# pangenome/povu

Measured on AMD Instinct MI355X. Metric: edges/sec decomposed (flubble+PVST), higher is better.
Workload: dtype u32

## Files before the change

include/povu_hip.h:

```cpp
#ifndef POVU_HIP_H
#define POVU_HIP_H

#include <stddef.h>
#include <stdint.h>

#ifdef __cplusplus
extern "C" {
#endif

#define POVU_HIP_NIL 0xFFFFFFFFu
#define POVU_SIDE_L 0
#define POVU_SIDE_R 1
#define POVU_TIP_NONE 0
#define POVU_TIP_L 1
#define POVU_TIP_R 2

typedef struct povu_hip_ctx povu_hip_ctx;
typedef struct povu_hip_forest povu_hip_forest;

int povu_hip_device_count(void);

povu_hip_ctx *povu_hip_create(int device, char *err, size_t errlen);
void povu_hip_destroy(povu_hip_ctx *ctx);
int povu_hip_release_workspace(povu_hip_ctx *ctx);
// ... 191 lines not shown
uint32_t povu_hip_last_seq_redo(const povu_hip_ctx *ctx);
int povu_hip_last_black_only_classes(const povu_hip_ctx *ctx);
int povu_hip_last_laminar_check_ran(const povu_hip_ctx *ctx);
int povu_hip_last_crossings(povu_hip_ctx *ctx, uint32_t out[2]);
uint64_t povu_hip_last_links_processed(const povu_hip_ctx *ctx);

int povu_hip_debug_components(povu_hip_ctx *ctx, uint32_t *comp_of, uint32_t *local_idx);
int povu_hip_debug_tree(povu_hip_ctx *ctx, uint32_t comp, uint32_t *n_tree, uint32_t *gid, uint8_t *typ,
			uint32_t *par, uint32_t *cls);
int povu_hip_debug_edge_ids(povu_hip_ctx *ctx, uint32_t comp, uint32_t *n_tree, uint32_t *tree_edge_id);
int povu_hip_debug_stack(povu_hip_ctx *ctx, uint32_t comp, uint32_t *n, uint32_t *tree_vtx, uint32_t *cls,
			 uint32_t *next_seen);

int povu_hip_debug_scan(povu_hip_ctx *ctx, int op, const uint32_t *in, uint32_t *out, size_t n, const uint32_t *in2,
			uint32_t *out2, size_t n2);
double povu_hip_debug_scan_time(povu_hip_ctx *ctx, size_t n, int reps, int op);

uint64_t povu_hip_workspace_estimate(uint32_t n_vtx, uint32_t n_links, uint32_t n_components);
int povu_hip_workspace_breakdown(uint32_t n_vtx, uint32_t n_links, uint32_t n_components, uint64_t out[7]);
int povu_hip_prewarm(povu_hip_ctx *ctx, uint32_t n_vtx, uint32_t n_links, char *err, size_t errlen);
uint64_t povu_hip_leaf_workspace_estimate(uint32_t n_vtx, uint32_t n_components);

const char *povu_hip_version(void);

#ifdef __cplusplus
}
#endif
#endif
```

povu_amd/csrc/hip/povu_hip.hip:

```cpp
#include "context.hpp"

#include <algorithm>
#include <atomic>
#include <cstdlib>
#include <memory>
#include <mutex>
#include <numeric>
#include <type_traits>

#include <fcntl.h>
#include <sys/mman.h>
#include <unistd.h>

using namespace povu_hip;

PinnedPool::~PinnedPool()
{
	for (auto &b : free_blocks)
		if (b.seg < 0)
			(void)hipHostFree(b.p);
	for (auto &sg : segments) {
		(void)hipHostUnregister(sg.p);
		(void)munmap(sg.p, sg.cap);
		(void)shm_unlink(segment_name(shared_tag, sg.seg).c_str());
// ... 1574 lines not shown
			scan_exclusive_u32_pair(di, dout, n, di2, dout2, n2, tmp, tb, s);
		else if (op == 0)
			scan_exclusive_u32(di, dout, n, tmp, tb, s);
		else
			scan_exclusive_max_u32(di, dout, n, tmp, tb, s);
		HIP_CHECK(copy_async(out, dout, n * 4, hipMemcpyDeviceToHost, s));
		if (in2 && op == 0)
			HIP_CHECK(copy_async(out2, dout2, n2 * 4, hipMemcpyDeviceToHost, s));
		HIP_CHECK(hipStreamSynchronize(s));
		return 0;
	} catch (const std::exception &) {
		return 2;
	}
}

extern "C" double povu_hip_debug_scan_time(povu_hip_ctx *ctx, size_t n, int reps, int op)
{
	if (!ctx || !n || reps <= 0)
		return -1.0;
	try {
		HIP_CHECK(hipSetDevice(ctx->device));
		hipStream_t s = ctx->stream;
		Arena ar;
		const size_t tb = scan_tmp_bytes(n);
		ar.reserve(2 * Arena::padded(n + 16, 4) + tb + 4096);
		uint32_t *di = ar.take<uint32_t>(n + 16), *dout = ar.take<uint32_t>(n + 16);
		void *tmp = ar.take<char>(tb);
		HIP_CHECK(hipMemsetAsync(di, 1, n * 4, s));
		hipEvent_t e0, e1;
		HIP_CHECK(hipEventCreate(&e0));
// ... 176 lines not shown
```

povu_amd/csrc/hip/tree_kernels.hip:

```cpp
#include "tree_kernels.hpp"

#include <cstdlib>

#include <algorithm>

namespace povu_hip
{

#ifndef NIL
#define NIL POVU_NIL
#endif
static constexpr int TPB = 256;
static inline unsigned nblk(size_t n) { return (unsigned)((n + TPB - 1) / TPB); }
#define LAUNCH(k, n, s, ...)                                                                     \
	do {                                                                                     \
		if ((n) > 0) {                                                                   \
			hipLaunchKernelGGL(k, dim3(nblk(n)), dim3(TPB), 0, s, __VA_ARGS__);      \
			HIP_CHECK(hipGetLastError());                                            \
		}                                                                                \
	} while (0)

static unsigned rank_bucket_bits(size_t n)
{
	if (const char *ev = getenv("POVU_HIP_RANK_BITS"))
// ... 242 lines not shown
	}
	return L0 ? heads[id - A.m] : A.hbase + (id - A.m);
}
template <bool EVT3>
__device__ __forceinline__ void rank_l0_weights(uint32_t x, uint32_t p, uint32_t &wa, uint32_t &wb)
{
	if (EVT3) {
		const uint32_t t = x % 3u;
		wa = t == 0 ? 2u : 0u;
		wb = t == 0 ? 2u : ((t == 1 && (p & P0_W)) ? 0u - 2u : 0u - 1u);
	} else {
		wa = (p & P0_W) ? 1u : 0u;
		wb = wa ? 1u : 0xFFFFFFFFu;
	}
}
template <bool L0, bool TWO, bool EVT3 = false>
__global__ void k_rank_up(RankLevelArgs A, unsigned b, const uint32_t *__restrict__ nx_in, const uint32_t *__restrict__ a_in,
			  const uint32_t *__restrict__ b_in, const uint32_t *__restrict__ heads, uint32_t *__restrict__ nx_out,
			  uint32_t *__restrict__ a_out, uint32_t *__restrict__ b_out)
{
	const uint32_t id = BIDX * blockDim.x + threadIdx.x;
	if (id >= A.M)
		return;
	uint32_t x = rank_lane_start<L0>(id, A, b, nx_in, heads);
	uint32_t sa = 0, sb = 0, out = PK_END | PK_STOP;
	if (x != NIL) {
		uint32_t p;
		bool stop;
		do {
			p = nx_in[x];
			if (L0) {
				uint32_t wa, wb;
				rank_l0_weights<EVT3>(x, p, wa, wb);
				sa += wa;
				if (TWO)
					sb += wb;
				x = p & P0_END;
				stop = rank_l0_stop(x, b);
			} else {
				sa += a_in[x];
				if (TWO)
					sb += b_in[x];
				x = p & PK_END;
				stop = (p & PK_STOP) != 0;
			}
		} while (!stop);
		if (x != (L0 ? P0_END : PK_END)) {
			const uint32_t q = x >> b;
			out = q | (is_splitter(q, b) ? PK_STOP : 0u);
		}
	}
	nx_out[id] = out;
	a_out[id] = sa;
	if (TWO)
		b_out[id] = sb;
}
template <bool L0, bool TWO, bool EVT3 = false>
__global__ void k_rank_down(RankLevelArgs A, unsigned b, const uint32_t *__restrict__ nx_in, uint32_t *a_io, uint32_t *b_io,
			    const uint32_t *__restrict__ heads, const uint32_t *__restrict__ ra, const uint32_t *__restrict__ rb,
			    uint32_t *__restrict__ out1, uint2 *__restrict__ out12)
{
	const uint32_t id = BIDX * blockDim.x + threadIdx.x;
	if (id >= A.M)
		return;
	uint32_t x = rank_lane_start<L0>(id, A, b, nx_in, heads);
	if (x == NIL)
		return;
	uint32_t sa = ra[id], sb = TWO ? rb[id] : 0, p;
	do {
		p = nx_in[x];
		if (L0) {
			uint32_t wa, wb;
			rank_l0_weights<EVT3>(x, p, wa, wb);
			if (TWO) {
				out12[x] = make_uint2(sa, sb);
				sb -= wb;
			} else {
				out1[x] = sa;
			}
			sa -= wa;
		} else {
			const uint32_t wa = a_io[x];
			a_io[x] = sa;
			sa -= wa;
			if (TWO) {
				const uint32_t wb = b_io[x];
				b_io[x] = sb;
				sb -= wb;
			}
		}
		if (L0) {
			x = p & P0_END;
			if (rank_l0_stop(x, b))
				break;
		} else {
			x = p & PK_END;
			if (p & PK_STOP)
				break;
		}
	} while (true);
}
template <bool TWO>
__global__ void __launch_bounds__(1024) k_rank_top(uint32_t n, const uint32_t *__restrict__ nx_in, uint32_t *a_io, uint32_t *b_io)
{
	__shared__ uint32_t nx[RANK_TOP], sa[RANK_TOP], sb[TWO ? RANK_TOP : 1];
	for (uint32_t i = threadIdx.x; i < n; i += blockDim.x) {
		const uint32_t p = nx_in[i] & PK_END;
		nx[i] = p == PK_END ? NIL : p;
		sa[i] = a_io[i];
		if (TWO)
			sb[i] = b_io[i];
	}
	__syncthreads();
	constexpr int PER = RANK_TOP / 1024;
	for (uint32_t span = 1; span < n; span <<= 1) {
// ... 35 lines not shown
	if (i < n) {
		const uint32_t p = nx_in[i] & PK_END;
		out[i] = p == PK_END ? NIL : p;
	}
}

struct RankBufs {
	uint32_t *pk;
	uint32_t *heads;
	uint32_t *nx, *wa, *wb;
	uint32_t *tA, *tB, *tC;
};
static constexpr int RANK_MAX_LEVELS = 12;
static size_t rank_pool_words(size_t n, size_t nh) { return n / 2 + 4 * nh + 64; }

template <bool TWO, bool EVT3 = false>
static void list_rank_splitters(uint32_t n, unsigned b, uint32_t *out1, uint2 *out12, uint32_t nh, RankBufs &rb, hipStream_t s)
{
	if (n >= P0_END)
		throw HipError("list ranking: more than 2^30 elements (graph too large for the packed walk)");
	RankLevelArgs lv[RANK_MAX_LEVELS];
	uint32_t *nxp[RANK_MAX_LEVELS + 1], *wap[RANK_MAX_LEVELS + 1], *wbp[RANK_MAX_LEVELS + 1];
	int levels = 0;
	size_t used = 0;
	const size_t pool = rank_pool_words(n, nh);
	nxp[0] = rb.pk, wap[0] = wbp[0] = nullptr;
	uint32_t cur_n = n, hbase = 0;
	for (;;) {
		RankLevelArgs &A = lv[levels];
		A.n = cur_n;
		A.m = (cur_n + (1u << b) - 1) >> b;
		A.hbase = hbase;
		A.M = A.m + nh;
		if (used + A.M > pool)
			throw HipError("list ranking: level pool exhausted (internal sizing bug)");
		nxp[levels + 1] = rb.nx + used, wap[levels + 1] = rb.wa + used, wbp[levels + 1] = rb.wb + used;
		used += A.M;
		levels++;
		hbase = A.m;
		const uint32_t next_n = A.M;
		if (next_n <= RANK_TOP || next_n > cur_n / 2 || levels == RANK_MAX_LEVELS) {
			cur_n = next_n;
			break;
		}
		cur_n = next_n;
	}
	for (int L = 0; L < levels; L++) {
		const RankLevelArgs &A = lv[L];
		if (L == 0)
			LAUNCH((k_rank_up<true, TWO, EVT3>), A.M, s, A, b, nxp[0], nullptr, nullptr, rb.heads, nxp[1], wap[1], wbp[1]);
		else
			LAUNCH((k_rank_up<false, TWO>), A.M, s, A, b, nxp[L], wap[L], wbp[L], nullptr, nxp[L + 1], wap[L + 1], wbp[L + 1]);
	}
	const uint32_t nt = cur_n;
	if (nt <= RANK_TOP) {
		KLAUNCH((k_rank_top<TWO>), dim3(1), dim3(1024), 0, s, nt, nxp[levels], wap[levels], wbp[levels]);
	} else {
		LAUNCH(k_rank_unpack_next, nt, s, nt, nxp[levels], rb.tA);
		HIP_CHECK(copy_async(rb.tB, wap[levels], (size_t)nt * 4, hipMemcpyDeviceToDevice, s));
		if (TWO)
			HIP_CHECK(copy_async(rb.tC, wbp[levels], (size_t)nt * 4, hipMemcpyDeviceToDevice, s));
		uint32_t *nA = rb.tA, *nB = nxp[levels], *aA = rb.tB, *aB = wap[levels], *bA = rb.tC, *bB = wbp[levels];
		const int side = list_rank(nt, bits_for(nt) + 1, nA, nB, aA, aB, TWO ? bA : nullptr, TWO ? bB : nullptr, s);
		if (side == 0) {
			HIP_CHECK(copy_async(wap[levels], aA, (size_t)nt * 4, hipMemcpyDeviceToDevice, s));
			if (TWO)
				HIP_CHECK(copy_async(wbp[levels], bA, (size_t)nt * 4, hipMemcpyDeviceToDevice, s));
		}
	}
	for (int L = levels - 1; L >= 0; L--) {
		const RankLevelArgs &A = lv[L];
		if (L == 0)
			LAUNCH((k_rank_down<true, TWO, EVT3>), A.M, s, A, b, nxp[0], nullptr, nullptr, rb.heads, wap[1], wbp[1], out1, out12);
		else
			LAUNCH((k_rank_down<false, TWO>), A.M, s, A, b, nxp[L], wap[L], wbp[L], nullptr, wap[L + 1], wbp[L + 1], nullptr,
			       nullptr);
	}
}

static constexpr uint32_t T0_RBIT = 0x80000000u;
__global__ void k_t0_parents(uint32_t V, const uint32_t *__restrict__ dist, const uint32_t *__restrict__ ckey,
			     const uint32_t *__restrict__ voff, const uint32_t *__restrict__ loff, const uint32_t *__restrict__ ladj,
			     const uint32_t *__restrict__ lle,
			     const uint32_t *__restrict__ ft, const uint32_t *__restrict__ heads,
			     uint4 *__restrict__ t0seg, uint4 *__restrict__ xrec, uint32_t C,
			     const unsigned long long *__restrict__ start_key, uint32_t *__restrict__ err, uint8_t *__restrict__ multi)
{
	uint32_t g = BIDX * blockDim.x + threadIdx.x;
	if (g < V)
		*reinterpret_cast<uint16_t *>(multi + 2 * g) = 0;
	if (g < C) {
		const uint32_t r = comp_root_side(start_key, voff, g), L = 2 * (voff[g + 1] - voff[g] - 1);
		t0seg[r >> 1] = make_uint4(NIL, (r & 1u) ? T0_RBIT : 0u, 0u, L ? L - 1 : 0u);
		const uint32_t h = heads[g];
		if (h == NIL ? L != 0 : dist[h] != L - 1)
			atomicExch(err, 1u);
	}
	if (g >= V)
		return;
	const uint32_t sb = loff[2 * g], sm = loff[2 * g + 1], se = loff[2 * g + 2];
	uint32_t at_e = NIL, dmin = 0xFFFFFFFFu, dmax = 0u;
	for (uint32_t at0 = sb; at0 < se; at0 += 4) {
		const uint4 lw4 = load4_unaligned(lle + at0), d4 = load4_unaligned(dist + at0);
		const uint32_t lws[4] = {lw4.x, lw4.y, lw4.z, lw4.w}, ds[4] = {d4.x, d4.y, d4.z, d4.w};
#pragma unroll
		for (uint32_t q = 0; q < 4; q++) {
			if (at0 + q >= se || !(lws[q] & LLE_TREE))
				continue;
			if (ds[q] < dmin) {
				dmin = ds[q];
				at_e = at0 + q;
			}
			dmax = max(dmax, ds[q]);
		}
	}
	if (at_e == NIL)
		return;
	const uint32_t c = ckey[g];
	if ((comp_root_side(start_key, voff, c) >> 1) == g)
		return;
	const uint32_t L = 2 * (voff[c + 1] - voff[c] - 1), abase = 2 * (voff[c] - c);
	const uint32_t p_in = abase + (L - 2 - dmax), p_out = abase + (L - 1 - dmin);
// ... 29 lines not shown
	const uint2 f2 = *reinterpret_cast<const uint2 *>(ft + 2 * g);
	if (!((f2.x | f2.y) & FT_HASH))
		return;
	const uint4 r = t0seg[g];
	if (r.x == NIL)
		return;
	const ulonglong2 z = make_ulonglong2(0ull, 0ull);
	xval[tour_rank(xrec, r.z)] = hx((f2.x & FT_HASH) ? hside[2 * g] : z, (f2.y & FT_HASH) ? hside[2 * g + 1] : z);
}
static constexpr uint32_t PB_BRIDGE = 0x80000000u;
static constexpr uint32_t CLASS_BUDGET = 256;
static constexpr uint32_t CS_VISITED = 0x40000000u;
__global__ void k_bridges(uint32_t V, const uint4 *__restrict__ t0seg, const ulonglong2 *__restrict__ xps,
			  const uint4 *__restrict__ xrec,
			  const ulonglong2 *__restrict__ hside, const uint32_t *__restrict__ ft,
			  const uint32_t *__restrict__ dist, const uint32_t *__restrict__ loff, const uint32_t *__restrict__ lle,
			  const uint32_t *__restrict__ ckey, const uint32_t *__restrict__ cproc, const uint32_t *__restrict__ voff,
			  uint8_t *multi, uint32_t *__restrict__ cstate, uint2 *__restrict__ dps)
{
	const uint32_t g = BIDX * blockDim.x + threadIdx.x;
	if (g >= V)
		return;
	auto stretch = [&](uint32_t p, uint32_t q) {
		const uint32_t rp = tour_rank(xrec, p), rq = tour_rank(xrec, q);
		return rp == rq ? make_ulonglong2(0ull, 0ull) : hx(xps[rp], xps[rq]);
	};
	const uint4 r = t0seg[g];
	const uint32_t Se = (2 * g) | (r.y >> 31), Sf = Se ^ 1u, c = ckey[g];
	const bool proc = cproc[c] != 0;
	uint32_t pvE;
	if (r.x == NIL) {
// ... 3 lines not shown
	} else {
		pvE = r.x;
		multi[Se] = 1;
		multi[r.x] = 1;
	}
	const uint2 f2 = *reinterpret_cast<const uint2 *>(ft + 2 * g);
	const uint32_t fF = (Sf & 1u) ? f2.y : f2.x, fE = (Sf & 1u) ? f2.x : f2.y, a1 = fF & FT_NONE;
	ulonglong2 x = (fF & FT_HASH) ? hside[Sf] : make_ulonglong2(0ull, 0ull);
	if (a1 != FT_NONE) {
		const uint32_t L = 2 * (voff[c + 1] - voff[c] - 1), abase = 2 * (voff[c] - c);
		const uint32_t a3 = fE & FT_NONE;
		uint32_t end;
		if (r.x == NIL)
			end = abase + L;
		else if (a3 != FT_NONE && (lle[a3] & LLE_ID) != (r.y & ~T0_RBIT))
			end = abase + (L - 1 - dist[a3]);
		else
			end = r.w;
		x = hx(x, stretch(abase + (L - 1 - dist[a1]), end));
	}
	uint32_t pvF;
	if (hzero(x)) {
		pvF = Se | PB_BRIDGE;
	} else {
		pvF = Se;
		multi[Sf] = 1;
		multi[Se] = 1;
	}
	const bool entryE = proc && (pvE & PB_BRIDGE), entryF = proc && (pvF & PB_BRIDGE);
	const uint32_t csE = proc ? (pvE | (entryE ? CS_VISITED : 0u)) : NIL, csF = proc ? (pvF | (entryF ? CS_VISITED : 0u)) : NIL;
	uint2 recE = make_uint2(NIL, 0u), recF = make_uint2(NIL, 0u);
	if (entryE && pvE != NIL) {
		const uint32_t p = pvE & ~PB_BRIDGE;
		recE.x = p;
// ... 452 lines not shown
			heads[comp] = A;
		}
	}
	pk[A] = enter;
	if (ns_o != NIL) {
		pk[A + 1] = rank_pack(3 * (ns_o >> 1), 0u, b);
		pk[A + 2] = rank_pack(after_e, 0u, b);
		merged[g] = 0;
	} else {
		pk[A + 1] = rank_pack(after_e, 1u, b);
		pk[A + 2] = P0_END;
		merged[g] = 1;
	}
}

__global__ void k_tree_emit(uint32_t nS, const uint2 *__restrict__ cd, const uint8_t *__restrict__ merged,
			    const uint2 *__restrict__ dps, const uint32_t *__restrict__ ckey,
			    const uint32_t *__restrict__ cproc, const uint32_t *__restrict__ voff,
			    const unsigned long long *__restrict__ start_key, const uint32_t *__restrict__ gid_s,
			    uint32_t *__restrict__ t_gid, uint8_t *__restrict__ t_flags, uint32_t *__restrict__ t_par,
			    uint32_t *__restrict__ t_size, uint32_t *__restrict__ t_depth, uint32_t *__restrict__ side_tidx,
			    uint32_t C, uint32_t *__restrict__ c_ntree, uint32_t *__restrict__ ordcnt, uint32_t *__restrict__ hi0,
			    uint32_t *__restrict__ mpre, uint32_t *__restrict__ srccnt, uint32_t *__restrict__ sdl,
			    uint32_t *__restrict__ incnt)
{
	uint32_t S = BIDX * blockDim.x + threadIdx.x;
	if (S == 0) {
		const uint32_t T = 2 * (nS >> 1) + C;
		hi0[T] = NIL;
		srccnt[T] = srccnt[T + 1] = 0;
		incnt[T] = incnt[T + 1] = 0;
// ... 28 lines not shown
	}
	const uint32_t g = S;
	if (g >= (nS >> 1))
		return;
	const uint32_t c = ckey[g], v0 = voff[c];
	const uint32_t tb = 2 * v0 + c;
	if (!cproc[c]) {
		const uint32_t t = tb + 2 * (g - v0);
		store2_unaligned(t_size + t, 0u, 0u);
		store2_unaligned(srccnt + t, 0u, 0u);
		store2_unaligned(incnt + t, 0u, 0u);
		*reinterpret_cast<uint2 *>(side_tidx + 2 * g) = make_uint2(NIL, NIL);
		return;
	}
	const uint32_t Nh = 2 * (voff[c + 1] - v0), hd = start_key[c] != ~0ull ? 1u : 0u;
	const uint4 cd01 = load4_unaligned(reinterpret_cast<const uint32_t *>(cd + 3 * g));
	const uint2 ent = make_uint2(cd01.x, cd01.y), lv_o = make_uint2(cd01.z, cd01.w);
	const uint4 d4 = *reinterpret_cast<const uint4 *>(dps + 2 * g);
	const uint32_t o = d4.x == 2 * g + 1 ? 2 * g : 2 * g + 1, e = o ^ 1u;
	const uint32_t p = (e & 1u) ? d4.z : d4.x;
	const uint32_t pre_e = Nh - ent.x, depth_e = 0u - ent.y;
	const uint32_t size_o = ent.x - 1 - lv_o.x, size_e = ent.x - (merged[g] ? lv_o.x : cd[3 * g + 2].x);
	uint32_t par_e;
	if (p == NIL)
		par_e = hd ? 0u : NIL;
	else
		par_e = hd + (Nh - cd[3 * (p >> 1)].x) + (dps[p].x == (p ^ 1u) ? 1u : 0u);
	const uint32_t l = hd + pre_e, t = tb + l;
	const uint32_t gid = gid_s[g];
	store2_unaligned(t_gid + t, gid, gid);
	t_flags[t] = (uint8_t)(e & 1u);
	t_flags[t + 1] = (uint8_t)((o & 1u) | TF_BLACK);
	store2_unaligned(t_par + t, par_e, l);
	store2_unaligned(t_size + t, size_e, size_o);
	store2_unaligned(incnt + t, 0u, 0u);
	if (t_depth)
		store2_unaligned(t_depth + t, depth_e + hd, depth_e + 1 + hd);
	store2_unaligned(mpre + t, tb + (depth_e + hd) + (Nh + hd) - l - size_e, tb + (depth_e + 1 + hd) + (Nh + hd) - (l + 1) - size_o);
	*reinterpret_cast<uint2 *>(side_tidx + 2 * g) = (e & 1u) ? make_uint2(t + 1, t) : make_uint2(t, t + 1);
	if (sdl) {
		const uint32_t gray = (size_e - 1 - size_o) / 2, black = (size_o + 1) / 2, gs = v0 + pre_e / 2;
		if (gray) {
// ... 242 lines not shown
static void tree_spans(TreeWs &tw, size_t V, size_t E, size_t Cmax, int groups, const StageWsOpts &o, F &&take_any)
{
	auto take1 = [&](void **p, size_t bytes) {
		if (groups & 1)
			take_any(p, bytes);
	};
	auto take = [&](void **p, size_t bytes) {
		if (groups & 2)
			take_any(p, bytes);
	};
	const size_t nS = 2 * V + 2, NA = std::max<size_t>(4 * V, 2 * E) + 8;
	const size_t NSL = std::max<size_t>(2 * V + 2 * E, 4 * V) + 16;
	take1((void **)&tw.dvis_slots, std::max(2 * E, 2 * V) + 16);
	take1((void **)&tw.side_tidx, nS * 4);
	take1((void **)&tw.dps, nS * 8);
	take((void **)&tw.dist, NSL * 4);
	take((void **)&tw.xrec, (NA / 64 + 4) * 16);
	take((void **)&tw.xrank, (NA / 64 + 4) * 4);
	take((void **)&tw.evt, NA * 8);
	take((void **)&tw.t0seg, (V + 2) * 16);
	for (uint32_t **p : {&tw.entry_ps, &tw.entry_list, &tw.be_cnt})
		take((void **)p, nS * 4);
	take((void **)&tw.dvis, nS);
	take((void **)&tw.wadj, (nS + 2 * E + 8) * 4);
	take((void **)&tw.cproc, (Cmax + 2) * 4);
	take((void **)&tw.rk_pk, NSL * 4);
	take((void **)&tw.rk_heads, (Cmax + 2) * 4);
	auto pad = [](size_t b) { return (b + 255) & ~size_t(255); };
	const size_t pool_b = pad(rank_pool_words(NSL, Cmax + 1) * 4);
	const size_t xv_b = pad((std::max<size_t>(V + 2, E + 8) + 8) * 16);
	const size_t wrec_b = pad(nS * 32);
// ... 77 lines not shown
{
	const uint32_t V = sw.V, E = sw.E, nS = 2 * V;
	const unsigned long long *start_key = (const unsigned long long *)cs.start_key;

	tm.begin("tree_root_forest");
	const uint32_t NA = 2 * (V - C);
	const size_t n_slots = 2 * (size_t)E;
	RankBufs rb{tw.rk_pk, tw.rk_heads, tw.rk_nx, tw.rk_wa, tw.rk_wb, tw.rk_tA, tw.rk_tB, tw.rk_tC};
	const unsigned bitsA = force_sparse_splitters ? 4u : rank_bucket_bits(n_slots);
	ulonglong2 *hside = reinterpret_cast<ulonglong2 *>(tw.evt);
	uint32_t *ft = tw.be_cnt;
	if (!tw.tour_words_done)
		tree_tour_words(cs, V, E, tw, force_sparse_splitters, s);
	tw.tour_words_done = false;
	LAUNCH(k_tour_ends, C, s, C, cs.voff, start_key, cs.loff, cs.ladj, cs.lle, rb.pk, rb.heads);
	if (n_slots)
		list_rank_splitters<false>((uint32_t)n_slots, bitsA, tw.dist, nullptr, C, rb, s);
	const uint32_t *dist = tw.dist;
	const uint32_t XW = NA / 64 + 1;
	HIP_CHECK(hipMemsetAsync(tw.xrec, 0, ((size_t)XW + 2) * 16, s));
	LAUNCH(k_t0_parents, std::max(V, C), s, V, dist, cs.ckey, cs.voff, cs.loff, cs.ladj, cs.lle, ft, rb.heads,
	       tw.t0seg, tw.xrec, C, start_key, pw.err + 2, tw.dvis_slots);
	tm.end(40);

	tm.begin("tree_bridges_classes");
	LAUNCH(k_bit_counts, (size_t)XW + 1, s, XW, tw.xrec, tw.xrank);
	scan_exclusive_u32(tw.xrank, tw.xrank, (size_t)XW + 1, pw.scan_tmp, pw.scan_tmp_bytes, s);
	LAUNCH(k_bit_ranks, XW, s, XW, tw.xrank, tw.xrec);
	LAUNCH(k_tour_values, V, s, V, tw.t0seg, ft, hside, tw.xrec, tw.xval);
	scan_exclusive_xor_u128(tw.xval, tw.xps, (size_t)V + 1, pw.scan_tmp, pw.scan_tmp_bytes, s, tw.xrank + XW);
	uint8_t *multi = tw.dvis_slots;
	uint32_t *cstate = sw.cur;
	LAUNCH(k_bridges, V, s, V, tw.t0seg, tw.xps, tw.xrec, hside, ft, dist, cs.loff, cs.lle, cs.ckey, tw.cproc, cs.voff, multi, cstate, tw.dps);
	tm.end(8 + 44);

	tm.begin("tree_class_dfs");
	uint32_t *n_entry_dev = pw.err + 9;
	KLAUNCH(k_entry_list, dim3((nS + EL_SIDES - 1) / EL_SIDES), dim3(TPB), 0, s, nS, cstate, multi, cs.ckey, tw.cproc, tw.entry_list, n_entry_dev);
	const uint32_t *big_list = tw.entry_list;
	const uint32_t n_events = 3 * V;
	const unsigned bitsE = force_sparse_splitters ? 4u : rank_bucket_bits(n_events);
	uint8_t *merged = tw.dvis;
	bool events_done = false;
	auto enqueue_events = [&]() {
		HIP_CHECK(hipMemsetAsync(rb.heads, 0xFF, (size_t)C * 4, s));
		LAUNCH(k_events, V, s, V, tw.dps, cs.loff, cs.ladj, cs.ckey, tw.cproc, rb.pk, rb.heads, bitsE, merged, pw.sdl);
	};
	uint32_t n_big = force_big_class_dfs ? tw.host->read_u32(n_entry_dev, s) : 0;
// ... 46 lines not shown
			walk_err, nS, route);
		if (s2 != s) {
			HIP_CHECK(hipEventRecord(tw.walk_join, s2));
			HIP_CHECK(hipStreamWaitEvent(s, tw.walk_join, 0));
		}
		LAUNCH(k_walk_finish, nS, s, nS, tw.wpar, cstate, cs.loff, cs.ladj, tw.dps);
		if (tw.host->read_u32(walk_err, s))
			throw HipError("class walk: stack pool exhausted (internal sizing bug)");
	}
	tm.end(5);

	tm.begin("tree_preorder");
	(void)max_side_links;
	if (!events_done)
		enqueue_events();
	list_rank_splitters<true, true>(n_events, bitsE, nullptr, tw.evt, C, rb, s);
	(void)event_lists;
	tm.end(40);

	tm.begin("tree_emit");
	LAUNCH(k_tree_emit, std::max(V, C), s, nS, tw.evt, merged, tw.dps, cs.ckey, tw.cproc, cs.voff, start_key, cs.gid_s, sw.t_gid, sw.t_flags,
	       sw.t_par, sw.t_size, (sw.hairpins || sw.want_depth) ? sw.t_depth : nullptr, tw.side_tidx, C, sw.c_ntree, pw.lsz, pw.hi0, pw.mpre, pw.dlt,
	       pw.sdl, pw.incnt);
	pw.sdl_filled = true;
	const uint8_t *dupflag = nullptr;
	if (max_side_links > 64 && E) {
		const uint32_t n_slots = 2 * E;
		uint32_t *k1 = (uint32_t *)tw.xval, *k2 = k1 + n_slots, *v1 = (uint32_t *)tw.xps, *v2 = v1 + n_slots;
		uint32_t *side_of = (uint32_t *)tw.evt;
		LAUNCH(k_slot_keys, n_slots, s, n_slots, cs.ladj, k1, v1);
		sort_pairs_u32(k1, k2, v1, v2, n_slots, bits_for(nS), pw.sort_tmp, pw.sort_tmp_bytes, s);
		LAUNCH(k_slot_side, nS, s, nS, cs.loff, side_of);
		LAUNCH(k_gather_keys, n_slots, s, n_slots, v2, side_of, k1);
		sort_pairs_u32(k1, k2, v2, v1, n_slots, bits_for(nS), pw.sort_tmp, pw.sort_tmp_bytes, s);
		LAUNCH(k_dup_flags, n_slots, s, n_slots, k2, v1, cs.ladj, tw.dvis_slots);
		dupflag = tw.dvis_slots;
// ... 12 lines not shown
```

povu_amd/csrc/hip/tree_kernels.hpp:

```cpp
#pragma once
#include "common.hpp"
#include "graph_kernels.hpp"
#include "par_kernels.hpp"
#include "seq_kernels.hpp"

namespace povu_hip
{

struct TreeWs {
	HostScratch *host;
	uint32_t *dist;
	ulonglong2 *xval, *xps;
	uint4 *xrec;
	uint32_t *xrank;
	uint4 *t0seg;
	uint2 *dps;
	uint8_t *dvis;
	uint32_t *wadj;
	uint4 *wrec;
	uint2 *wstk;
	uint32_t *wpar;
	uint8_t *dvis_slots;
	uint32_t *entry_ps, *entry_list;
	uint32_t *side_tidx;
	uint32_t *be_cnt;
	uint32_t *rk_pk, *rk_heads;
// ... 8 lines not shown
	bool walk_inline = true;
};

size_t tree_workspace_bytes(size_t V, size_t E, size_t Cmax, int groups = 3, const StageWsOpts &o = StageWsOpts{});
void tree_carve(Arena &ar, TreeWs &tw, size_t V, size_t E, size_t Cmax, int groups = 3, const StageWsOpts &o = StageWsOpts{});
size_t stage_workspace_bytes(size_t V, size_t E, size_t Cmax, const StageWsOpts &o = StageWsOpts{});
void stage_workspace_carve(Arena &ar, ParWs &pw, TreeWs &tw, size_t V, size_t E, size_t Cmax, const StageWsOpts &o = StageWsOpts{});
size_t walk_workspace_bytes(size_t V);

void tree_tour_words(const CompState &cs, uint32_t V, uint32_t E, TreeWs &tw, bool force_sparse_splitters, hipStream_t s);

int64_t run_parallel_tree(const CompState &cs, SeqWs &sw, ParWs &pw, TreeWs &tw, uint32_t C, uint32_t event_lists,
			   uint32_t max_side_links, bool force_big_class_dfs, bool force_sparse_splitters, StageTimer &tm,
			   hipStream_t s);

void debug_edge_id_weights(const CompState &cs, const SeqWs &sw, const TreeWs &tw, uint32_t *w, uint32_t *tail, hipStream_t s);

}
```

povu_amd/hip.py:

```python
from __future__ import annotations

import ctypes as C
import os
from dataclasses import dataclass
from typing import Dict, List, Optional

import numpy as np

_HERE = os.path.dirname(os.path.abspath(__file__))


class HipUnavailable(RuntimeError):
    pass


def lib_path() -> str:
    return os.path.join(_HERE, "lib", "libpovu_hip.so")


class _Opts(C.Structure):
    _fields_ = [("rank", C.c_uint32), ("world", C.c_uint32), ("flags", C.c_uint32)]


class _SubTree(C.Structure):
# ... 121 lines not shown
    l.povu_hip_last_black_only_classes.restype = C.c_int
    l.povu_hip_last_black_only_classes.argtypes = [C.c_void_p]
    l.povu_hip_last_crossings.restype = C.c_int
    l.povu_hip_last_crossings.argtypes = [C.c_void_p, C.POINTER(C.c_uint32)]
    l.povu_hip_last_laminar_check_ran.restype = C.c_int
    l.povu_hip_last_laminar_check_ran.argtypes = [C.c_void_p]
    l.povu_hip_debug_edge_ids.restype = C.c_int
    l.povu_hip_debug_edge_ids.argtypes = [C.c_void_p, C.c_uint32, C.POINTER(C.c_uint32), C.c_void_p]
    l.povu_hip_debug_stack.restype = C.c_int
    l.povu_hip_debug_stack.argtypes = [C.c_void_p, C.c_uint32, C.POINTER(C.c_uint32), C.c_void_p, C.c_void_p,
                                       C.c_void_p]
    l.povu_hip_version.restype = C.c_char_p
    l.povu_hip_debug_scan.restype = C.c_int
    l.povu_hip_debug_scan.argtypes = [C.c_void_p, C.c_int, C.c_void_p, C.c_void_p, C.c_size_t, C.c_void_p, C.c_void_p,
                                      C.c_size_t]
    l.povu_hip_workspace_estimate.restype = C.c_uint64
    l.povu_hip_workspace_estimate.argtypes = [C.c_uint32, C.c_uint32, C.c_uint32]
    l.povu_hip_prewarm.restype = C.c_int
    l.povu_hip_prewarm.argtypes = [C.c_void_p, C.c_uint32, C.c_uint32, C.c_char_p, C.c_size_t]
    l.povu_hip_leaf_workspace_estimate.restype = C.c_uint64
    l.povu_hip_leaf_workspace_estimate.argtypes = [C.c_uint32, C.c_uint32]
    l.povu_hip_lpt_assign.restype = C.c_int
    l.povu_hip_lpt_assign.argtypes = [C.c_void_p, C.c_uint32, C.c_uint32, C.c_void_p]
    l.povu_hip_shard_partition.restype = C.c_void_p
    l.povu_hip_shard_partition.argtypes = [C.c_void_p, C.c_uint32, C.c_char_p, C.c_size_t]
    l.povu_hip_shards_world.restype = C.c_uint32
    l.povu_hip_shards_world.argtypes = [C.c_void_p]
    l.povu_hip_shards_total_components.restype = C.c_uint32
    l.povu_hip_shards_total_components.argtypes = [C.c_void_p]
    l.povu_hip_shards_get.restype = C.c_int
# ... 464 lines not shown
        a = np.ascontiguousarray(a, dtype=np.uint32)
        out = np.empty_like(a)
        if b is None:
            rc = self._lib.povu_hip_debug_scan(self._ctx, op, a.ctypes.data, out.ctypes.data, a.size, None, None, 0)
            if rc:
                raise RuntimeError(f"debug_scan failed ({rc})")
            return out
        b = np.ascontiguousarray(b, dtype=np.uint32)
        out2 = np.empty_like(b)
        rc = self._lib.povu_hip_debug_scan(self._ctx, op, a.ctypes.data, out.ctypes.data, a.size, b.ctypes.data,
                                           out2.ctypes.data, b.size)
        if rc:
            raise RuntimeError(f"debug_scan failed ({rc})")
        return out, out2

    def debug_components(self, n_vtx: int):
        comp = np.zeros(n_vtx, dtype=np.uint32)
        loc = np.zeros(n_vtx, dtype=np.uint32)
        if self._lib.povu_hip_debug_components(self._ctx, comp.ctypes.data, loc.ctypes.data) != 0:
            raise RuntimeError("no decompose state")
        return comp, loc

    def debug_tree(self, comp: int):
        n = C.c_uint32(0)
        if self._lib.povu_hip_debug_tree(self._ctx, comp, C.byref(n), None, None, None, None) != 0:
            raise RuntimeError("no decompose state")
        gid = np.zeros(n.value, dtype=np.uint32)
        typ = np.zeros(n.value, dtype=np.uint8)
        par = np.zeros(n.value, dtype=np.uint32)
        cls = np.zeros(n.value, dtype=np.uint32)
# ... 100 lines not shown
```

Measured before the change: 3.005 billion.

## Record splitter-relative offsets in rank-up and drop level-0 rank-down pass

```diff
diff --git a/include/povu_hip.h b/include/povu_hip.h
--- a/include/povu_hip.h
+++ b/include/povu_hip.h
@@ -229,6 +229,8 @@
 
 int povu_hip_debug_scan(povu_hip_ctx *ctx, int op, const uint32_t *in, uint32_t *out, size_t n, const uint32_t *in2,
 			uint32_t *out2, size_t n2);
+int povu_hip_debug_list_rank(povu_hip_ctx *ctx, uint32_t n, const uint32_t *next, const uint8_t *w, const uint32_t *heads,
+			     uint32_t nh, int mode, uint32_t bits, uint32_t *ra, uint32_t *rb);
 double povu_hip_debug_scan_time(povu_hip_ctx *ctx, size_t n, int reps, int op);
 
 uint64_t povu_hip_workspace_estimate(uint32_t n_vtx, uint32_t n_links, uint32_t n_components);
diff --git a/povu_amd/csrc/hip/povu_hip.hip b/povu_amd/csrc/hip/povu_hip.hip
--- a/povu_amd/csrc/hip/povu_hip.hip
+++ b/povu_amd/csrc/hip/povu_hip.hip
@@ -1612,6 +1612,20 @@
 	}
 }
 
+extern "C" int povu_hip_debug_list_rank(povu_hip_ctx *ctx, uint32_t n, const uint32_t *next, const uint8_t *w, const uint32_t *heads,
+					uint32_t nh, int mode, uint32_t bits, uint32_t *ra, uint32_t *rb)
+{
+	if (!ctx || !next || !w || (nh && !heads) || !ra || (mode != 0 && !rb) || mode < 0 || mode > 1)
+		return 1;
+	try {
+		HIP_CHECK(hipSetDevice(ctx->device));
+		debug_list_rank(n, next, w, heads, nh, mode, bits, ra, rb, ctx->stream);
+		return 0;
+	} catch (const std::exception &) {
+		return 2;
+	}
+}
+
 extern "C" double povu_hip_debug_scan_time(povu_hip_ctx *ctx, size_t n, int reps, int op)
 {
 	if (!ctx || !n || reps <= 0)
diff --git a/povu_amd/csrc/hip/tree_kernels.hip b/povu_amd/csrc/hip/tree_kernels.hip
--- a/povu_amd/csrc/hip/tree_kernels.hip
+++ b/povu_amd/csrc/hip/tree_kernels.hip
@@ -3,6 +3,7 @@
 #include <cstdlib>
 
 #include <algorithm>
+#include <vector>
 
 namespace povu_hip
 {
@@ -280,16 +281,18 @@
 		wb = wa ? 1u : 0xFFFFFFFFu;
 	}
 }
+static constexpr uint32_t REC_MAX = 0xFFFFu;
 template <bool L0, bool TWO, bool EVT3 = false>
 __global__ void k_rank_up(RankLevelArgs A, unsigned b, const uint32_t *__restrict__ nx_in, const uint32_t *__restrict__ a_in,
 			  const uint32_t *__restrict__ b_in, const uint32_t *__restrict__ heads, uint32_t *__restrict__ nx_out,
-			  uint32_t *__restrict__ a_out, uint32_t *__restrict__ b_out)
+			  uint32_t *__restrict__ a_out, uint32_t *__restrict__ b_out, uint2 *__restrict__ rec, uint32_t *__restrict__ ovf)
 {
 	const uint32_t id = BIDX * blockDim.x + threadIdx.x;
 	if (id >= A.M)
 		return;
 	uint32_t x = rank_lane_start<L0>(id, A, b, nx_in, heads);
 	uint32_t sa = 0, sb = 0, out = PK_END | PK_STOP;
+	bool big = false;
 	if (x != NIL) {
 		uint32_t p;
 		bool stop;
@@ -298,6 +301,12 @@
 			if (L0) {
 				uint32_t wa, wb;
 				rank_l0_weights<EVT3>(x, p, wa, wb);
+				if (TWO) {
+					big |= sa > REC_MAX || sa - sb > REC_MAX;
+					rec[x] = make_uint2(id, sa | ((sa - sb) << 16));
+				} else {
+					rec[x] = make_uint2(id, sa);
+				}
 				sa += wa;
 				if (TWO)
 					sb += wb;
@@ -320,51 +329,55 @@
 	a_out[id] = sa;
 	if (TWO)
 		b_out[id] = sb;
-}
-template <bool L0, bool TWO, bool EVT3 = false>
+	if (L0 && TWO && big)
+		*ovf = 1u;
+}
+template <bool EVT3>
+__global__ void k_rank_l0_fallback(RankLevelArgs A, unsigned b, const uint32_t *__restrict__ pk, const uint32_t *__restrict__ heads,
+				   const uint32_t *__restrict__ ra, const uint32_t *__restrict__ rb, uint2 *__restrict__ rec,
+				   const uint32_t *__restrict__ ovf)
+{
+	if (!*ovf)
+		return;
+	for (uint32_t id = BIDX * blockDim.x + threadIdx.x; id < A.M; id += gridDim.x * blockDim.x) {
+		uint32_t x = rank_lane_start<true>(id, A, b, pk, heads);
+		if (x == NIL)
+			continue;
+		uint32_t sa = ra[id], sb = rb[id];
+		do {
+			const uint32_t p = pk[x];
+			uint32_t wa, wb;
+			rank_l0_weights<EVT3>(x, p, wa, wb);
+			rec[x] = make_uint2(sa, sb);
+			sa -= wa;
+			sb -= wb;
+			x = p & P0_END;
+		} while (!rank_l0_stop(x, b));
+	}
+}
+template <bool TWO>
 __global__ void k_rank_down(RankLevelArgs A, unsigned b, const uint32_t *__restrict__ nx_in, uint32_t *a_io, uint32_t *b_io,
-			    const uint32_t *__restrict__ heads, const uint32_t *__restrict__ ra, const uint32_t *__restrict__ rb,
-			    uint32_t *__restrict__ out1, uint2 *__restrict__ out12)
+			    const uint32_t *__restrict__ ra, const uint32_t *__restrict__ rb)
 {
 	const uint32_t id = BIDX * blockDim.x + threadIdx.x;
 	if (id >= A.M)
 		return;
-	uint32_t x = rank_lane_start<L0>(id, A, b, nx_in, heads);
+	uint32_t x = rank_lane_start<false>(id, A, b, nx_in, nullptr);
 	if (x == NIL)
 		return;
 	uint32_t sa = ra[id], sb = TWO ? rb[id] : 0, p;
 	do {
 		p = nx_in[x];
-		if (L0) {
-			uint32_t wa, wb;
-			rank_l0_weights<EVT3>(x, p, wa, wb);
-			if (TWO) {
-				out12[x] = make_uint2(sa, sb);
-				sb -= wb;
-			} else {
-				out1[x] = sa;
-			}
-			sa -= wa;
-		} else {
-			const uint32_t wa = a_io[x];
-			a_io[x] = sa;
-			sa -= wa;
-			if (TWO) {
-				const uint32_t wb = b_io[x];
-				b_io[x] = sb;
-				sb -= wb;
-			}
-		}
-		if (L0) {
-			x = p & P0_END;
-			if (rank_l0_stop(x, b))
-				break;
-		} else {
-			x = p & PK_END;
-			if (p & PK_STOP)
-				break;
-		}
-	} while (true);
+		const uint32_t wa = a_io[x];
+		a_io[x] = sa;
+		sa -= wa;
+		if (TWO) {
+			const uint32_t wb = b_io[x];
+			b_io[x] = sb;
+			sb -= wb;
+		}
+		x = p & PK_END;
+	} while (!(p & PK_STOP));
 }
 template <bool TWO>
 __global__ void __launch_bounds__(1024) k_rank_top(uint32_t n, const uint32_t *__restrict__ nx_in, uint32_t *a_io, uint32_t *b_io)
@@ -430,8 +443,29 @@
 static constexpr int RANK_MAX_LEVELS = 12;
 static size_t rank_pool_words(size_t n, size_t nh) { return n / 2 + 4 * nh + 64; }
 
+struct L0Ranks {
+	const uint32_t *ra, *rb, *fin;
+	uint32_t M;
+};
+__device__ __forceinline__ uint32_t rank_l0(const L0Ranks &R, uint2 rec)
+{
+	return (rec.x < R.M ? R.ra[rec.x] : 0u) - rec.y;
+}
+__device__ __forceinline__ uint32_t rank_l0_a(const L0Ranks &R, uint2 rec, bool fin)
+{
+	return fin ? rec.x : (rec.x < R.M ? R.ra[rec.x] : 0u) - (rec.y & REC_MAX);
+}
+__device__ __forceinline__ uint2 rank_l0_pair(const L0Ranks &R, uint2 rec, bool fin)
+{
+	if (fin)
+		return rec;
+	const bool in = rec.x < R.M;
+	const uint32_t ra = in ? R.ra[rec.x] : 0u, rb = in ? R.rb[rec.x] : 0u, pa = rec.y & REC_MAX;
+	return make_uint2(ra - pa, rb - pa + (rec.y >> 16));
+}
+
 template <bool TWO, bool EVT3 = false>
-static void list_rank_splitters(uint32_t n, unsigned b, uint32_t *out1, uint2 *out12, uint32_t nh, RankBufs &rb, hipStream_t s)
+static L0Ranks list_rank_splitters(uint32_t n, unsigned b, uint2 *rec, uint32_t *ovf, uint32_t nh, RankBufs &rb, hipStream_t s)
 {
 	if (n >= P0_END)
 		throw HipError("list ranking: more than 2^30 elements (graph too large for the packed walk)");
@@ -461,12 +495,15 @@
 		}
 		cur_n = next_n;
 	}
+	if (TWO)
+		HIP_CHECK(hipMemsetAsync(ovf, 0, 4, s));
 	for (int L = 0; L < levels; L++) {
 		const RankLevelArgs &A = lv[L];
 		if (L == 0)
-			LAUNCH((k_rank_up<true, TWO, EVT3>), A.M, s, A, b, nxp[0], nullptr, nullptr, rb.heads, nxp[1], wap[1], wbp[1]);
+			LAUNCH((k_rank_up<true, TWO, EVT3>), A.M, s, A, b, nxp[0], nullptr, nullptr, rb.heads, nxp[1], wap[1], wbp[1], rec, ovf);
 		else
-			LAUNCH((k_rank_up<false, TWO>), A.M, s, A, b, nxp[L], wap[L], wbp[L], nullptr, nxp[L + 1], wap[L + 1], wbp[L + 1]);
+			LAUNCH((k_rank_up<false, TWO>), A.M, s, A, b, nxp[L], wap[L], wbp[L], nullptr, nxp[L + 1], wap[L + 1], wbp[L + 1],
+			       nullptr, nullptr);
 	}
 	const uint32_t nt = cur_n;
 	if (nt <= RANK_TOP) {
@@ -484,18 +521,76 @@
 				HIP_CHECK(copy_async(wbp[levels], bA, (size_t)nt * 4, hipMemcpyDeviceToDevice, s));
 		}
 	}
-	for (int L = levels - 1; L >= 0; L--) {
+	for (int L = levels - 1; L >= 1; L--) {
 		const RankLevelArgs &A = lv[L];
-		if (L == 0)
-			LAUNCH((k_rank_down<true, TWO, EVT3>), A.M, s, A, b, nxp[0], nullptr, nullptr, rb.heads, wap[1], wbp[1], out1, out12);
-		else
-			LAUNCH((k_rank_down<false, TWO>), A.M, s, A, b, nxp[L], wap[L], wbp[L], nullptr, wap[L + 1], wbp[L + 1], nullptr,
-			       nullptr);
-	}
+		LAUNCH((k_rank_down<TWO>), A.M, s, A, b, nxp[L], wap[L], wbp[L], wap[L + 1], wbp[L + 1]);
+	}
+	if (TWO)
+		KLAUNCH((k_rank_l0_fallback<EVT3>), dim3(std::min(nblk(lv[0].M), 2048u)), dim3(TPB), 0, s, lv[0], b, rb.pk, rb.heads, wap[1],
+			wbp[1], rec, ovf);
+	return L0Ranks{wap[1], TWO ? wbp[1] : nullptr, TWO ? ovf : nullptr, lv[0].M};
+}
+
+template <bool TWO>
+__global__ void k_rank_resolve(uint32_t n, const uint2 *__restrict__ rec, L0Ranks R, uint32_t *__restrict__ ra, uint32_t *__restrict__ rb)
+{
+	const uint32_t x = BIDX * blockDim.x + threadIdx.x;
+	if (x >= n)
+		return;
+	if (TWO) {
+		const uint2 r = rank_l0_pair(R, rec[x], *R.fin != 0);
+		ra[x] = r.x;
+		rb[x] = r.y;
+	} else {
+		ra[x] = rank_l0(R, rec[x]);
+	}
+}
+void debug_list_rank(uint32_t n, const uint32_t *next, const uint8_t *w, const uint32_t *heads, uint32_t nh, int mode,
+		     unsigned bits, uint32_t *ra, uint32_t *rb, hipStream_t s)
+{
+	if (n == 0 || n >= P0_END)
+		throw HipError("debug_list_rank: n must be in [1, 2^30)");
+	const unsigned b = bits ? std::min(6u, std::max(2u, bits)) : rank_bucket_bits(n);
+	std::vector<uint32_t> pk(n);
+	for (uint32_t x = 0; x < n; x++) {
+		if (next[x] != NIL && next[x] >= n)
+			throw HipError("debug_list_rank: successor out of range");
+		pk[x] = (next[x] == NIL ? P0_END : next[x]) | (w[x] ? P0_W : 0u);
+	}
+	for (uint32_t h = 0; h < nh; h++)
+		if (heads[h] != NIL) {
+			if (heads[h] >= n)
+				throw HipError("debug_list_rank: head out of range");
+			pk[heads[h]] |= P0_HEAD;
+		}
+	const size_t pool = rank_pool_words(n, nh);
+	Arena ar;
+	ar.reserve(Arena::padded(n + 16, 4) * 3 + Arena::padded(n + 16, 8) + Arena::padded(nh + 1, 4) + 6 * Arena::padded(pool, 4) + 8192, false);
+	RankBufs rbf{};
+	rbf.pk = ar.take<uint32_t>(n + 16);
+	rbf.heads = ar.take<uint32_t>(nh + 1);
+	for (uint32_t **q : {&rbf.nx, &rbf.wa, &rbf.wb, &rbf.tA, &rbf.tB, &rbf.tC})
+		*q = ar.take<uint32_t>(pool);
+	uint32_t *da = ar.take<uint32_t>(n + 16), *db = ar.take<uint32_t>(n + 16), *ovf = ar.take<uint32_t>(4);
+	uint2 *rec = ar.take<uint2>(n + 16);
+	HIP_CHECK(copy_async(rbf.pk, pk.data(), (size_t)n * 4, hipMemcpyHostToDevice, s));
+	if (nh)
+		HIP_CHECK(copy_async(rbf.heads, heads, (size_t)nh * 4, hipMemcpyHostToDevice, s));
+	if (mode == 0) {
+		const L0Ranks R = list_rank_splitters<false>(n, b, rec, nullptr, nh, rbf, s);
+		LAUNCH(k_rank_resolve<false>, n, s, n, rec, R, da, nullptr);
+	} else {
+		const L0Ranks R = list_rank_splitters<true, true>(n, b, rec, ovf, nh, rbf, s);
+		LAUNCH(k_rank_resolve<true>, n, s, n, rec, R, da, db);
+	}
+	HIP_CHECK(copy_async(ra, da, (size_t)n * 4, hipMemcpyDeviceToHost, s));
+	if (mode != 0)
+		HIP_CHECK(copy_async(rb, db, (size_t)n * 4, hipMemcpyDeviceToHost, s));
+	HIP_CHECK(hipStreamSynchronize(s));
 }
 
 static constexpr uint32_t T0_RBIT = 0x80000000u;
-__global__ void k_t0_parents(uint32_t V, const uint32_t *__restrict__ dist, const uint32_t *__restrict__ ckey,
+__global__ void k_t0_parents(uint32_t V, const uint2 *__restrict__ trec, L0Ranks R, const uint32_t *__restrict__ ckey,
 			     const uint32_t *__restrict__ voff, const uint32_t *__restrict__ loff, const uint32_t *__restrict__ ladj,
 			     const uint32_t *__restrict__ lle,
 			     const uint32_t *__restrict__ ft, const uint32_t *__restrict__ heads,
@@ -509,7 +604,7 @@
 		const uint32_t r = comp_root_side(start_key, voff, g), L = 2 * (voff[g + 1] - voff[g] - 1);
 		t0seg[r >> 1] = make_uint4(NIL, (r & 1u) ? T0_RBIT : 0u, 0u, L ? L - 1 : 0u);
 		const uint32_t h = heads[g];
-		if (h == NIL ? L != 0 : dist[h] != L - 1)
+		if (h == NIL ? L != 0 : rank_l0(R, trec[h]) != L - 1)
 			atomicExch(err, 1u);
 	}
 	if (g >= V)
@@ -517,11 +612,20 @@
 	const uint32_t sb = loff[2 * g], sm = loff[2 * g + 1], se = loff[2 * g + 2];
 	uint32_t at_e = NIL, dmin = 0xFFFFFFFFu, dmax = 0u;
 	for (uint32_t at0 = sb; at0 < se; at0 += 4) {
-		const uint4 lw4 = load4_unaligned(lle + at0), d4 = load4_unaligned(dist + at0);
-		const uint32_t lws[4] = {lw4.x, lw4.y, lw4.z, lw4.w}, ds[4] = {d4.x, d4.y, d4.z, d4.w};
+		const uint32_t *r32 = reinterpret_cast<const uint32_t *>(trec + at0);
+		const uint4 lw4 = load4_unaligned(lle + at0), r01 = load4_unaligned(r32), r23 = load4_unaligned(r32 + 4);
+		const uint32_t lws[4] = {lw4.x, lw4.y, lw4.z, lw4.w};
+		const uint2 rs[4] = {make_uint2(r01.x, r01.y), make_uint2(r01.z, r01.w), make_uint2(r23.x, r23.y), make_uint2(r23.z, r23.w)};
+		bool tree[4];
+		uint32_t ds[4];
 #pragma unroll
 		for (uint32_t q = 0; q < 4; q++) {
-			if (at0 + q >= se || !(lws[q] & LLE_TREE))
+			tree[q] = at0 + q < se && (lws[q] & LLE_TREE);
+			ds[q] = tree[q] ? rank_l0(R, rs[q]) : 0u;
+		}
+#pragma unroll
+		for (uint32_t q = 0; q < 4; q++) {
+			if (!tree[q])
 				continue;
 			if (ds[q] < dmin) {
 				dmin = ds[q];
@@ -581,7 +685,7 @@
 __global__ void k_bridges(uint32_t V, const uint4 *__restrict__ t0seg, const ulonglong2 *__restrict__ xps,
 			  const uint4 *__restrict__ xrec,
 			  const ulonglong2 *__restrict__ hside, const uint32_t *__restrict__ ft,
-			  const uint32_t *__restrict__ dist, const uint32_t *__restrict__ loff, const uint32_t *__restrict__ lle,
+			  const uint2 *__restrict__ trec, L0Ranks R, const uint32_t *__restrict__ loff, const uint32_t *__restrict__ lle,
 			  const uint32_t *__restrict__ ckey, const uint32_t *__restrict__ cproc, const uint32_t *__restrict__ voff,
 			  uint8_t *multi, uint32_t *__restrict__ cstate, uint2 *__restrict__ dps)
 {
@@ -615,10 +719,10 @@
 		if (r.x == NIL)
 			end = abase + L;
 		else if (a3 != FT_NONE && (lle[a3] & LLE_ID) != (r.y & ~T0_RBIT))
-			end = abase + (L - 1 - dist[a3]);
+			end = abase + (L - 1 - rank_l0(R, trec[a3]));
 		else
 			end = r.w;
-		x = hx(x, stretch(abase + (L - 1 - dist[a1]), end));
+		x = hx(x, stretch(abase + (L - 1 - rank_l0(R, trec[a1])), end));
 	}
 	uint32_t pvF;
 	if (hzero(x)) {
@@ -1101,7 +1205,7 @@
 	}
 }
 
-__global__ void k_tree_emit(uint32_t nS, const uint2 *__restrict__ cd, const uint8_t *__restrict__ merged,
+__global__ void k_tree_emit(uint32_t nS, const uint2 *__restrict__ erec, L0Ranks R, const uint8_t *__restrict__ merged,
 			    const uint2 *__restrict__ dps, const uint32_t *__restrict__ ckey,
 			    const uint32_t *__restrict__ cproc, const uint32_t *__restrict__ voff,
 			    const unsigned long long *__restrict__ start_key, const uint32_t *__restrict__ gid_s,
@@ -1160,18 +1264,25 @@
 		return;
 	}
 	const uint32_t Nh = 2 * (voff[c + 1] - v0), hd = start_key[c] != ~0ull ? 1u : 0u;
-	const uint4 cd01 = load4_unaligned(reinterpret_cast<const uint32_t *>(cd + 3 * g));
-	const uint2 ent = make_uint2(cd01.x, cd01.y), lv_o = make_uint2(cd01.z, cd01.w);
+	const bool fin = *R.fin != 0;
+	const uint4 r01 = load4_unaligned(reinterpret_cast<const uint32_t *>(erec + 3 * g));
+	const uint2 ent = rank_l0_pair(R, make_uint2(r01.x, r01.y), fin);
+	const uint2 lv_o = make_uint2(rank_l0_a(R, make_uint2(r01.z, r01.w), fin), 0u);
 	const uint4 d4 = *reinterpret_cast<const uint4 *>(dps + 2 * g);
 	const uint32_t o = d4.x == 2 * g + 1 ? 2 * g : 2 * g + 1, e = o ^ 1u;
 	const uint32_t p = (e & 1u) ? d4.z : d4.x;
 	const uint32_t pre_e = Nh - ent.x, depth_e = 0u - ent.y;
-	const uint32_t size_o = ent.x - 1 - lv_o.x, size_e = ent.x - (merged[g] ? lv_o.x : cd[3 * g + 2].x);
+	uint32_t lv_e = lv_o.x;
+	if (!merged[g]) {
+		lv_e = rank_l0_a(R, erec[3 * g + 2], fin);
+	}
+	const uint32_t size_o = ent.x - 1 - lv_o.x, size_e = ent.x - lv_e;
 	uint32_t par_e;
 	if (p == NIL)
 		par_e = hd ? 0u : NIL;
-	else
-		par_e = hd + (Nh - cd[3 * (p >> 1)].x) + (dps[p].x == (p ^ 1u) ? 1u : 0u);
+	else {
+		par_e = hd + (Nh - rank_l0_a(R, erec[3 * (p >> 1)], fin)) + (dps[p].x == (p ^ 1u) ? 1u : 0u);
+	}
 	const uint32_t l = hd + pre_e, t = tb + l;
 	const uint32_t gid = gid_s[g];
 	store2_unaligned(t_gid + t, gid, gid);
@@ -1444,7 +1555,7 @@
 	take1((void **)&tw.dvis_slots, std::max(2 * E, 2 * V) + 16);
 	take1((void **)&tw.side_tidx, nS * 4);
 	take1((void **)&tw.dps, nS * 8);
-	take((void **)&tw.dist, NSL * 4);
+	take((void **)&tw.dist, (2 * E + 16) * 8);
 	take((void **)&tw.xrec, (NA / 64 + 4) * 16);
 	take((void **)&tw.xrank, (NA / 64 + 4) * 4);
 	take((void **)&tw.evt, NA * 8);
@@ -1552,12 +1663,12 @@
 		tree_tour_words(cs, V, E, tw, force_sparse_splitters, s);
 	tw.tour_words_done = false;
 	LAUNCH(k_tour_ends, C, s, C, cs.voff, start_key, cs.loff, cs.ladj, cs.lle, rb.pk, rb.heads);
+	L0Ranks tour_r{};
 	if (n_slots)
-		list_rank_splitters<false>((uint32_t)n_slots, bitsA, tw.dist, nullptr, C, rb, s);
-	const uint32_t *dist = tw.dist;
+		tour_r = list_rank_splitters<false>((uint32_t)n_slots, bitsA, tw.dist, nullptr, C, rb, s);
 	const uint32_t XW = NA / 64 + 1;
 	HIP_CHECK(hipMemsetAsync(tw.xrec, 0, ((size_t)XW + 2) * 16, s));
-	LAUNCH(k_t0_parents, std::max(V, C), s, V, dist, cs.ckey, cs.voff, cs.loff, cs.ladj, cs.lle, ft, rb.heads,
+	LAUNCH(k_t0_parents, std::max(V, C), s, V, tw.dist, tour_r, cs.ckey, cs.voff, cs.loff, cs.ladj, cs.lle, ft, rb.heads,
 	       tw.t0seg, tw.xrec, C, start_key, pw.err + 2, tw.dvis_slots);
 	tm.end(40);
 
@@ -1569,7 +1680,7 @@
 	scan_exclusive_xor_u128(tw.xval, tw.xps, (size_t)V + 1, pw.scan_tmp, pw.scan_tmp_bytes, s, tw.xrank + XW);
 	uint8_t *multi = tw.dvis_slots;
 	uint32_t *cstate = sw.cur;
-	LAUNCH(k_bridges, V, s, V, tw.t0seg, tw.xps, tw.xrec, hside, ft, dist, cs.loff, cs.lle, cs.ckey, tw.cproc, cs.voff, multi, cstate, tw.dps);
+	LAUNCH(k_bridges, V, s, V, tw.t0seg, tw.xps, tw.xrec, hside, ft, tw.dist, tour_r, cs.loff, cs.lle, cs.ckey, tw.cproc, cs.voff, multi, cstate, tw.dps);
 	tm.end(8 + 44);
 
 	tm.begin("tree_class_dfs");
@@ -1646,12 +1757,12 @@
 	(void)max_side_links;
 	if (!events_done)
 		enqueue_events();
-	list_rank_splitters<true, true>(n_events, bitsE, nullptr, tw.evt, C, rb, s);
+	const L0Ranks evr = list_rank_splitters<true, true>(n_events, bitsE, tw.evt, pw.err + 13, C, rb, s);
 	(void)event_lists;
 	tm.end(40);
 
 	tm.begin("tree_emit");
-	LAUNCH(k_tree_emit, std::max(V, C), s, nS, tw.evt, merged, tw.dps, cs.ckey, tw.cproc, cs.voff, start_key, cs.gid_s, sw.t_gid, sw.t_flags,
+	LAUNCH(k_tree_emit, std::max(V, C), s, nS, tw.evt, evr, merged, tw.dps, cs.ckey, tw.cproc, cs.voff, start_key, cs.gid_s, sw.t_gid, sw.t_flags,
 	       sw.t_par, sw.t_size, (sw.hairpins || sw.want_depth) ? sw.t_depth : nullptr, tw.side_tidx, C, sw.c_ntree, pw.lsz, pw.hi0, pw.mpre, pw.dlt,
 	       pw.sdl, pw.incnt);
 	pw.sdl_filled = true;
diff --git a/povu_amd/csrc/hip/tree_kernels.hpp b/povu_amd/csrc/hip/tree_kernels.hpp
--- a/povu_amd/csrc/hip/tree_kernels.hpp
+++ b/povu_amd/csrc/hip/tree_kernels.hpp
@@ -9,7 +9,7 @@
 
 struct TreeWs {
 	HostScratch *host;
-	uint32_t *dist;
+	uint2 *dist;
 	ulonglong2 *xval, *xps;
 	uint4 *xrec;
 	uint32_t *xrank;
@@ -48,6 +48,9 @@
 			   uint32_t max_side_links, bool force_big_class_dfs, bool force_sparse_splitters, StageTimer &tm,
 			   hipStream_t s);
 
+void debug_list_rank(uint32_t n, const uint32_t *next, const uint8_t *w, const uint32_t *heads, uint32_t nh, int mode,
+		     unsigned bits, uint32_t *ra, uint32_t *rb, hipStream_t s);
+
 void debug_edge_id_weights(const CompState &cs, const SeqWs &sw, const TreeWs &tw, uint32_t *w, uint32_t *tail, hipStream_t s);
 
 }
diff --git a/povu_amd/hip.py b/povu_amd/hip.py
--- a/povu_amd/hip.py
+++ b/povu_amd/hip.py
@@ -159,6 +159,9 @@
     l.povu_hip_debug_scan.restype = C.c_int
     l.povu_hip_debug_scan.argtypes = [C.c_void_p, C.c_int, C.c_void_p, C.c_void_p, C.c_size_t, C.c_void_p, C.c_void_p,
                                       C.c_size_t]
+    l.povu_hip_debug_list_rank.restype = C.c_int
+    l.povu_hip_debug_list_rank.argtypes = [C.c_void_p, C.c_uint32, C.c_void_p, C.c_void_p, C.c_void_p, C.c_uint32,
+                                           C.c_int, C.c_uint32, C.c_void_p, C.c_void_p]
     l.povu_hip_workspace_estimate.restype = C.c_uint64
     l.povu_hip_workspace_estimate.argtypes = [C.c_uint32, C.c_uint32, C.c_uint32]
     l.povu_hip_prewarm.restype = C.c_int
@@ -653,6 +656,19 @@
             raise RuntimeError(f"debug_scan failed ({rc})")
         return out, out2
 
+    def debug_list_rank(self, nxt, w, heads, events: bool = False, bits: int = 0):
+        nxt = np.ascontiguousarray(nxt, dtype=np.uint32)
+        w = np.ascontiguousarray(w, dtype=np.uint8)
+        heads = np.ascontiguousarray(heads, dtype=np.uint32)
+        ra = np.zeros(nxt.size, dtype=np.uint32)
+        rb = np.zeros(nxt.size, dtype=np.uint32)
+        rc = self._lib.povu_hip_debug_list_rank(self._ctx, nxt.size, nxt.ctypes.data, w.ctypes.data,
+                                                heads.ctypes.data if heads.size else None, heads.size,
+                                                1 if events else 0, bits, ra.ctypes.data, rb.ctypes.data)
+        if rc:
+            raise RuntimeError(f"debug_list_rank failed ({rc})")
+        return (ra, rb) if events else ra
+
     def debug_components(self, n_vtx: int):
         comp = np.zeros(n_vtx, dtype=np.uint32)
         loc = np.zeros(n_vtx, dtype=np.uint32)
```

Result: faster. 3.084 billion, median of 6 (+2.6%).
